# raznem/spp-rl

Hardware: AMD Instinct MI355X
Metric: env-steps/sec (rollout+update) SPP-SAC Hopper-v2 (higher is better)
Workload: dtype fp32

## Files before the change

include/spprl.h:

```cpp
#ifndef SPPRL_H
#define SPPRL_H
#include <stdint.h>

#ifdef __cplusplus
extern "C" {
#endif

typedef int sppStatus;
enum {
  SPP_OK = 0,
  SPP_E_INVALID_ARG = 1,
  SPP_E_SHAPE = 2,
  SPP_E_OOM = 3,
  SPP_E_HIP = 4,
  SPP_E_STATE = 5,
  SPP_E_RCCL = 6
};

const char* sppGetLastError(void);
int sppGetVersion(void);

typedef struct sppMT19937* sppMTHandle;
sppStatus sppMTCreate(sppMTHandle* out, uint32_t seed);
sppStatus sppMTRandint(sppMTHandle h, int64_t high, int64_t n, int64_t* out_host);
// ... 113 lines not shown
sppStatus sppDdpgAcmCriticGrads(sppAgentHandle h, const sppBatch* batch, float* losses_dev, void* stream);
sppStatus sppDdpgAcmCriticApply(sppAgentHandle h, void* stream);
sppStatus sppDdpgAcmActorGrads(sppAgentHandle h, float* losses_dev, void* stream);
sppStatus sppDdpgAcmActorApply(sppAgentHandle h, void* stream);

#define SPP_COMM_ID_BYTES 128
sppStatus sppCommGetUniqueId(void* uid_out);
sppStatus sppCommInitRank(void** comm_out, int nranks, const void* uid, int rank, int device);
sppStatus sppCommDestroy(void* comm);
enum { SPP_BUCKET_CRITIC = 0, SPP_BUCKET_ACTOR = 1, SPP_BUCKET_ACM = 2, SPP_BUCKET_ALL = 3 };
sppStatus sppAllReduceGrads(sppAgentHandle h, int bucket, int world, void* rccl_comm, void* stream);
sppStatus sppCommAllReduceSum(void* rccl_comm, void* buf_dev, int64_t count, int dtype, void* stream);
sppStatus sppCommAllGather(void* rccl_comm, const void* send_dev, void* recv_dev, int64_t bytes, void* stream);

sppStatus sppAcmRegressStep(sppAgentHandle h, const float* x, const float* y, int B, float* loss_dev,
                            void* stream);
sppStatus sppAcmRegressGrads(sppAgentHandle h, const float* x, const float* y, int B, float* loss_dev,
                             void* stream);
sppStatus sppAcmRegressApply(sppAgentHandle h, void* stream);
sppStatus sppAcmSgd(sppAgentHandle h, const float* x_dev, const float* y_dev, int nsteps, int bs, float* loss_sum,
                    void* stream);
sppStatus sppAcmSgdEpoch(sppAgentHandle h, const float* x_dev, const float* y_dev, int nrows, int bs,
                         float* loss_sum, void* stream);
sppStatus sppAcmSgdStatus(sppAgentHandle h, int* timed_out_host);
sppStatus sppAcmSgdStatusAsync(sppAgentHandle h, int* timed_out_pinned, void* stream);
int sppAcmSgdMaxBatch(sppAgentHandle h);
int sppAcmSgdWorkgroups(sppAgentHandle h, int bs);
sppStatus sppReplayGatherAcm(sppReplayHandle h, const int64_t* idx_dev, int B, float* x, float* y, void* stream);
sppStatus sppReplaySetAcmColumns(sppReplayHandle h, const int* cols_host, int n);

sppStatus sppAgentSetTiming(sppAgentHandle h, int enable);
sppStatus sppAgentStageSplit(sppAgentHandle h, int* bits_out);
sppStatus sppAgentCriticPairs(sppAgentHandle h, int* bits_out);
sppStatus sppAgentGetTiming(sppAgentHandle h, double* ms_out , int64_t* count_out );

sppStatus sppPolicyAct(sppAgentHandle h, const float* obs , int E, const float* eps ,
                       const float* noise , float act_noise, int mode, int denormalize_actor_out,
                       float* target_state_out , float* env_action_out , void* stream);

sppStatus sppSynthEnvStep(const float* A , const float* obs , const float* action ,
                          int E, int ob, int ac, float* next_obs, float* reward, void* stream);

sppStatus sppRandUniform(float* out_dev, int64_t n, const float* lo_dev, const float* hi_dev, int period,
                         uint64_t seed, uint64_t offset, void* stream);
sppStatus sppEpisodeAccum(const float* rew, const uint8_t* end, int E, float* ep_ret, double* sums, void* stream);
sppStatus sppSynthEnvReset(float* obs , const uint8_t* mask, int E, int ob, uint64_t seed,
                           uint64_t offset, void* stream);

sppStatus sppObsNormalize(const float* x, int64_t rows, int ob, const float* lo, const float* hi, const float* mean,
                          const float* std, int min_max, int inverse, float* out, void* stream);

sppStatus sppGaeScan(const float* rew, const float* v, const float* v_next, const uint8_t* done,
                     const uint8_t* end, int64_t T, int64_t E, double gamma, double lam, int mode, float* q_out,
                     float* adv, void* stream);
sppStatus sppPpoClipLoss(const float* lp_old, const float* lp_new, const float* adv, int B, float eps, float* grad,
                         float* out2, void* stream);
sppStatus sppAdvNormalize(const float* adv, int64_t n, float* out, void* stream);
sppStatus sppAdvSums(const float* adv, int64_t n, double* sums2, void* stream);
sppStatus sppAdvNormalizeGlobal(const float* adv, int64_t n_local, const double* sums2, int64_t n_global, float* out,
                                void* stream);

typedef struct sppOnPolicy* sppOnPolicyHandle;
typedef struct {
  int ob, aout;
  float actor_lr, critic_lr;
  float ppo_epsilon;
// ... 51 lines not shown
```

spp-rl_amd/csrc/api.hip:

```cpp
#include <dlfcn.h>
#include <stdarg.h>
#include <stdio.h>
#include <string.h>

#include <algorithm>
#include <memory>
#include <string>
#include <vector>

#include "../../include/spprl.h"
#include "internal.h"
#include "layout.h"
#include "replay.h"
#include "sac_kernels.h"
#include "host.h"

#include "optim.hip"
#include "replay.hip"
#include "stats.hip"
#include "sac.hip"
#include "ddpg.hip"
#include "kset.h"
#ifdef SPP_SINGLE_TU
#include "ks_dw.hip"
// ... 1026 lines not shown
    }
    D.j0[0] = 0;
    D.nj[0] = (int)jobs.size();
  }
  if (a->cfg.mlp_bf16) {
    std::vector<const float*> b16;
    if (!a->ddpg && set == 0)
      b16 = {a->H1[0], a->H1[1], a->H2[0], a->H2[1], a->D1[0], a->D1[1], a->D2[0], a->D2[1],
             a->AH1, a->AH2, a->AD1, a->AD2};
    auto is16 = [&](const float* p) { return p && std::find(b16.begin(), b16.end(), p) != b16.end(); };
    for (DwJob& j : jobs) {
      j.bf16 = 1;
      j.a_bf = is16(j.A) ? 1 : 0;
      j.x_bf = is16(j.X0) ? 1 : 0;
    }
  }
  const sppStatus s = finalize_dw(D, jobs, nph, Bp, B, a->num_cu);
  if (set == 0) {
    for (int i = 0; i < 2; ++i) {
      const int f = fused[a->ddpg ? 0 : i];
      a->w3p[i] = f >= 0 ? jobs[f].slab : nullptr;
    }
    a->w3p_stride = fused[0] >= 0 ? jobs[fused[0]].slab_stride : 0;
  }
  return s;
}

namespace spp {

void launch_dw_set(DwSet& D, int ph, hipStream_t st) {
  const int* ij = D.items.ptr + D.ioff[ph];
  const int* is = ij + D.nitems[ph];
  const DwJob* jobs = D.jobs.ptr + D.j0[ph];
  launch_dw_kernels(jobs, ij, is, D.nitems[ph], D.nlds[ph], D.nj[ph], D.max_elems[ph], D.bf16, st);
}

int g_sgd_spin = 0;

constexpr int kSgdSyncInts = kSgdShardStride * (1 + kSgdShards);
int* sgd_ctr(DevArray<int>& sync) { return sync.ptr + kSgdShardStride; }
sppStatus mlp_sgd_buffers(DevArray<float>& slab, DevArray<int>& sync, hipStream_t st) {
  if (!slab.ptr) {
    SPP_CHECK_HIP(slab.alloc((size_t)(2 * kMlMaxWG + kSgdPubReps) * kMlSlabMax));
    SPP_CHECK_HIP(sync.alloc(kSgdSyncInts));
    SPP_CHECK_HIP(hipMemsetAsync(sync.ptr, 0, kSgdSyncInts * sizeof(int), st));
  }
  SPP_CHECK_HIP(hipMemsetAsync(sgd_ctr(sync), 0, kSgdShards * kSgdShardStride * sizeof(int), st));
  return SPP_OK;
}

void launch_pack_matrix(int gx, int njobs, const PackJob* jobs, hipStream_t st) {
  hipLaunchKernelGGL(k_pack_matrix, dim3(gx, njobs), dim3(256), 0, st, jobs);
}
void launch_adam_kernel(const AdamJob* job, int64_t n, float neg_step, float bc2s, hipStream_t st) {
  hipLaunchKernelGGL(k_adam, dim3(std::max(1, std::min(cdiv(n, 1024), 1024)), 1), dim3(256), 0, st, job, neg_step,
                     bc2s, 0.f);
}

}

static void launch_dw(sppAgent* a, int set, int ph, hipStream_t st) { launch_dw_set(a->dws[set], ph, st); }

static sppStatus build_adam(sppAgent* a) {
  AdamJob jobs[4] = {};
  for (int i = 0; i < (a->ddpg ? 1 : 2); ++i) {
    NetBufs& n = a->net[SPP_NET_CRITIC1 + i];
    jobs[i] = AdamJob{n.p, n.g, n.m, n.v, a->net[SPP_NET_CRITIC1_TARG + i].p, n.n};
  }
  NetBufs& na = a->net[SPP_NET_ACTOR];
  jobs[2] = AdamJob{na.p, na.g, na.m, na.v, a->ddpg ? a->net[SPP_NET_ACTOR_TARG].p : nullptr, na.n};
  NetBufs& nm = a->net[SPP_NET_ACM];
  jobs[3] = AdamJob{nm.p, nm.g, nm.m, nm.v, nullptr, nm.n};
  if (!a->d_adam.ptr) SPP_CHECK_HIP(a->d_adam.alloc(4));
  SPP_CHECK_HIP(hipMemcpy(a->d_adam.ptr, jobs, sizeof(jobs), hipMemcpyHostToDevice));
  return SPP_OK;
}

static void launch_adam(sppAgent* a, int first, int count, int64_t n, int64_t step, float lr, float tau,
                        hipStream_t st) {
  const double bc1 = 1.0 - std::pow(0.9, (double)step), bc2s = std::sqrt(1.0 - std::pow(0.999, (double)step));
  hipLaunchKernelGGL(k_adam, dim3(std::max(1, std::min(cdiv(n, 256 * 4), 1024)), count), dim3(256), 0, st,
                     (const AdamJob*)(a->d_adam.ptr + first), (float)(-(lr / bc1)), (float)bc2s, tau);
}

constexpr int kStageWGPerCU = 3;
constexpr int kStageSplitAll = 7;
constexpr int kStageSplitDefault = kStageSplitAll;
constexpr int kCriticPairsDefault = 1;
static int stage_grid(sppAgent* a, int Bp) {
  return std::max(1, std::min(cdiv(Bp / 32, kWavesPerWG), kStageWGPerCU * a->num_cu));
}

static SacArgs make_args(sppAgent* a, int B) {
  SacArgs p{};
  p.B = B;
  p.Bp = (int)round_up(B, 32);
  p.inv_B = 1.f / (float)B;
  p.S = a->S; p.S2 = a->S2; p.ACT = a->ACT; p.AENV = a->AENV; p.R = a->R; p.DN = a->DN;
  p.EPS1 = a->EPS1; p.EPS2 = a->EPS2;
  p.min_max = a->cfg.min_max_denormalize;
  p.lo = a->lo; p.hi = a->hi; p.mean = a->mean; p.std = a->std;
  p.actor_lim = a->limits.ptr;
  p.acm_lim = a->limits.ptr + a->cfg.aout;
  p.gamma = a->cfg.gamma;
  p.custom_loss = a->cfg.custom_loss;
  p.norm_closs = a->cfg.norm_closs;
  p.alpha = a->alpha_f32;
  p.actor = a->actor;
  for (int i = 0; i < 2; ++i) {
    p.critic[i] = a->critic[i];
    p.targ[i] = a->targ[i];
    p.H1[i] = a->H1[i]; p.H2[i] = a->H2[i]; p.D1[i] = a->D1[i]; p.D2[i] = a->D2[i]; p.DQ[i] = a->DQ[i];
    p.W3P[i] = a->w3p[i];
  }
  p.w3p_stride = a->w3p_stride;
  p.acm = a->acm;
  p.bacm = a->bacm;
  p.actor_targ = a->actor_targ;
  p.AH1 = a->AH1; p.AH2 = a->AH2; p.AD1 = a->AD1; p.AD2 = a->AD2; p.ADH = a->ADH;
  p.part = a->part;
  p.THD = a->THD; p.SCA = a->SCA; p.SLP = a->SLP;
// ... 59 lines not shown
  SPP_REQUIRE(cfg->algo != SPP_ALGO_SAC || (cfg->acm_critic == 0 && cfg->aout == cfg->ac && cfg->custom_loss == 0.f),
              SPP_E_INVALID_ARG, "vanilla SAC: the actor emits the env action (aout == ac), no ACM critic / loss");
  SPP_REQUIRE(cfg->algo != SPP_ALGO_DDPG || (cfg->acm_critic == 0 && cfg->aout == cfg->ac && cfg->custom_loss == 0.f),
              SPP_E_INVALID_ARG, "vanilla DDPG: the actor emits the env action (aout == ac), no ACM critic / loss");
  SPP_REQUIRE(cfg->algo != SPP_ALGO_DDPG || cfg->mlp_bf16 == 0, SPP_E_INVALID_ARG, "vanilla DDPG: fp32 only");
  SPP_REQUIRE(cfg->max_batch > 0, SPP_E_INVALID_ARG, "max_batch must be > 0");
  KernelSet ks;
  SPP_REQUIRE(find_kset(cfg->algo, cfg->ob, cfg->aout, cfg->ac, cfg->acm_critic != 0, cfg->mlp_bf16 != 0, &ks),
              SPP_E_SHAPE, "no kernel instantiation for algo %d (ob=%d, aout=%d, ac=%d, bf16=%d)", cfg->algo, cfg->ob,
              cfg->aout, cfg->ac, cfg->mlp_bf16);
  SPP_CHECK_HIP(hipSetDevice(device));
  auto a = std::make_unique<sppAgent>();
  a->cfg = *cfg;
  a->device = device;
  a->ks = ks;
  hipDeviceProp_t prop;
  SPP_CHECK_HIP(hipGetDeviceProperties(&prop, device));
  a->num_cu = prop.multiProcessorCount;
  {
    const char* t = getenv("SPP_SAC_TEAM");
    a->team_ok = !(t && t[0] == '0');
    const char* m = getenv("SPP_MINQ_SPLIT");
    a->minq_split = ks.actor_fwd && ks.actor_minq && ks.actor_bwd && !(m && m[0] == '0');
    const char* g = getenv("SPP_STAGE_SPLIT");
    const int want = g ? atoi(g) : kStageSplitDefault;
    const bool tab_fits = 128 + 3 * round_up(std::max(cfg->aout, 1), 32) + round_up(std::max(cfg->ac, 1), 32) <= kStageTab;
    const bool have = ks.heads_stage && ks.trunk_bwd && ks.trunk_fwd_a && ks.squash_a && ks.critics_a &&
                      ks.trunk_fwd_c && ks.squash_c && ks.critic_rest;
    if (a->minq_split && have && tab_fits) a->stage_split = want & kStageSplitAll;
    const char* cp = getenv("SPP_CRITIC_PAIRS");
    const int wantp = cp ? atoi(cp) : kCriticPairsDefault;
    if ((a->stage_split & 4) && ks.critic_rest_pair) a->critic_pairs |= wantp & 1;
    if ((a->stage_split & 2) && ks.critics_a_pair) a->critic_pairs |= wantp & 2;
  }
  const int ob = cfg->ob, aout = cfg->aout, ac = cfg->ac;
  a->cin = ob + (cfg->acm_critic ? ac : aout);
  a->ddpg = cfg->algo == SPP_ALGO_DDPG_ACM || cfg->algo == SPP_ALGO_DDPG;
  a->plain = cfg->algo == SPP_ALGO_SAC || cfg->algo == SPP_ALGO_DDPG;
  const bool dd = a->ddpg;
  a->lay[SPP_NET_ACTOR] = dd ? ddpg_actor_layout(ob, aout) : sac_actor_layout(ob, aout);
  if (dd) a->lay[SPP_NET_ACTOR_TARG] = a->lay[SPP_NET_ACTOR];
  a->lay[SPP_NET_CRITIC1] = a->lay[SPP_NET_CRITIC1_TARG] = critic_layout(a->cin);
  if (!dd) a->lay[SPP_NET_CRITIC2] = a->lay[SPP_NET_CRITIC2_TARG] = critic_layout(a->cin);
  if (!dd) a->lay[SPP_NET_ACM] = acm_layout(2 * ob, ac);
  else if (!a->plain) a->lay[SPP_NET_ACM] = bacm_layout(2 * ob, ac);
  a->Bmax = cfg->max_batch;
  const int64_t Bp = round_up(cfg->max_batch, 32);
  SPP_REQUIRE((int64_t)Bp * 256 * 4 < ((int64_t)1 << 31), SPP_E_SHAPE, "max_batch %d too large (31-bit buffer offsets)",
              cfg->max_batch);
  a->Bpmax = (int)Bp;
  const int64_t ntiles = Bp / 32;
  const int64_t per = Bp;
  int64_t total = 0;
  auto take = [&](int64_t rows) { int64_t o = total; total += rows * per; return o; };
  const int64_t oS = take(ob), oS2 = take(ob), oACT = take(aout), oAENV = take(ac), oR = take(1), oDN = take(1),
                oE1 = take(aout), oE2 = take(aout);
  int64_t oH1[2] = {}, oH2[2] = {}, oD1[2] = {}, oD2[2] = {}, oDQ[2] = {};
  for (int i = 0; i < (dd ? 1 : 2); ++i) {
    oH1[i] = take(256); oH2[i] = take(256); oD1[i] = take(256); oD2[i] = take(256); oDQ[i] = take(1);
  }
  const int64_t oAH1 = take(256), oAH2 = take(256), oAD1 = take(256), oAD2 = take(256), oADH = take(2 * aout);
  const int64_t oZ1 = take(dd ? 128 : 64), oZ2 = take(dd ? 64 : 32), oT3 = take(ac);
  const int64_t oRX = take(2 * ob), oRZ1 = take(dd ? 128 : 64), oRZ2 = take(dd ? 64 : 32), oRP1 = take(dd ? 128 : 64),
                oRP2 = take(dd ? 64 : 32), oRP3 = take(ac);
  const int64_t oRS21 = dd ? take(64) : 0, oRPZ21 = dd ? take(64) : 0;
  const int64_t oGAD = take(aout), oMASK = take(16);
// ... 234 lines not shown
  }
  tmark(a, 1, st);
  SPP_CHECK_HIP(hipGetLastError());
  tmark(a, 2, st);
  launch_dw(a, 0, 1, st);
  tmark(a, 2, st);
  hipLaunchKernelGGL(k_actor_partials, dim3(1), dim3(kFinThreads), 0, st, (const float*)a->part, p.Bp / 32, B, a->cfg.aout,
                     a->cfg.custom_loss, (double)a->cfg.target_entropy, a->alpha_grad ? a->alpha_grad : a->aux,
                     losses);
  SPP_CHECK_HIP(hipGetLastError());
  return SPP_OK;
}

sppStatus sppSacAcmActorGrads(sppAgentHandle a, const float* eps_cur, float* losses, void* stream) {
  SPP_REQUIRE(a, SPP_E_INVALID_ARG, "null");
  const int B = a->cur_B;
  SPP_REQUIRE(B > 0, SPP_E_STATE, "no staged batch");
  const int Bp = (int)round_up(B, 32);
  if (eps_cur)
    hipLaunchKernelGGL(k_eps_copy_fm, dim3(cdiv((int64_t)a->cfg.aout * Bp, 256)), dim3(256), 0, S(stream), eps_cur,
                       a->EPS2, a->cfg.aout, B, Bp);
  return actor_grads(a, losses, S(stream));
}

sppStatus sppAgentStageSplit(sppAgentHandle a, int* bits_out) {
  SPP_REQUIRE(a && bits_out, SPP_E_INVALID_ARG, "null");
  *bits_out = a->stage_split;
  return SPP_OK;
}

sppStatus sppAgentCriticPairs(sppAgentHandle a, int* bits_out) {
  SPP_REQUIRE(a && bits_out, SPP_E_INVALID_ARG, "null");
  *bits_out = a->critic_pairs;
  return SPP_OK;
}

sppStatus sppAgentBindAlphaGrad(sppAgentHandle a, float* g) {
  SPP_REQUIRE(a, SPP_E_INVALID_ARG, "null");
  a->alpha_grad = g;
  return SPP_OK;
}

sppStatus sppSacAcmDrawEps(sppAgentHandle a, uint64_t seed, uint64_t counter, void* stream) {
  SPP_REQUIRE(a && a->cur_B > 0, SPP_E_STATE, "no staged batch");
  const int B = a->cur_B, Bp = (int)round_up(B, 32);
  SPP_REQUIRE((int64_t)a->cfg.aout * Bp < ((int64_t)1 << 31), SPP_E_SHAPE, "draw_eps: aout * Bp >= 2^31");
  const int64_t quads = (int64_t)a->cfg.aout * Bp / 4;
  hipLaunchKernelGGL(k_eps_fm, dim3(cdiv(quads, 256), 2), dim3(256), 0, S(stream), a->EPS1, a->cfg.aout, B, Bp, seed,
                     2 * counter, a->EPS2, 2 * counter + 1);
  SPP_CHECK_HIP(hipGetLastError());
  return SPP_OK;
}

sppStatus sppAgentReadEps(sppAgentHandle a, int which, float* out, void* stream) {
  SPP_REQUIRE(a && out && (which == 0 || which == 1), SPP_E_INVALID_ARG, "read_eps: bad args");
  SPP_REQUIRE(a->cur_B > 0, SPP_E_STATE, "no staged batch");
  const int B = a->cur_B, Bp = (int)round_up(B, 32);
  hipLaunchKernelGGL(k_eps_read_fm, dim3(cdiv((int64_t)a->cfg.aout * B, 256)), dim3(256), 0, S(stream),
                     (const float*)(which ? a->EPS2 : a->EPS1), out, a->cfg.aout, B, Bp);
  SPP_CHECK_HIP(hipGetLastError());
  return SPP_OK;
}

static std::vector<PackJob> images_of(sppAgent* a, int net) {
  std::vector<PackJob> out;
  const NetBufs& nb = a->net[net];
// ... 611 lines not shown
```

spp-rl_amd/csrc/dw.hip:

```cpp
#include "common.h"
#include "internal.h"

namespace spp {

constexpr int kDwThreads = 256;

template <int NI, int NJ, bool BF = false, bool ABF = false, bool XBF = false>
constexpr int dw_ring() {
  constexpr int cyc = NI * NJ * (BF ? 32 : 512);
  constexpr int want = 1 + (8192 + cyc - 1) / cyc;
  constexpr int cap = 168 / (4 * (NI * (ABF ? 1 : 2) + NJ * (XBF ? 1 : 2)));
  constexpr int r = want < cap ? want : cap;
  return r < 2 ? 2 : (r > 8 ? 8 : r);
}

__device__ __forceinline__ bf16x8 pack8(const float4& a, const float4& b) {
  bf16x8 r;
  r[0] = (__bf16)a.x; r[1] = (__bf16)a.y; r[2] = (__bf16)a.z; r[3] = (__bf16)a.w;
  r[4] = (__bf16)b.x; r[5] = (__bf16)b.y; r[6] = (__bf16)b.z; r[7] = (__bf16)b.w;
  return r;
}

__device__ __forceinline__ bf16x8 as_bf8(const float4& a) { return __builtin_bit_cast(bf16x8, a); }
__device__ __forceinline__ float sum_bf8(const float4& a) {
// ... 51 lines not shown
      if constexpr (BF) {
        static_for<0, NI>([&](auto I) {
          if constexpr (DB && ABF) {
            bs[I] += sum_bf8(ra[u][I][0]);
          } else if constexpr (DB) {
            const float4 a0 = ra[u][I][0], a1 = ra[u][I][1];
            bs[I] += ((a0.x + a0.y) + (a0.z + a0.w)) + ((a1.x + a1.y) + (a1.z + a1.w));
          }
          const bf16x8 av = ABF ? as_bf8(ra[u][I][0]) : pack8(ra[u][I][0], ra[u][I][1]);
          static_for<0, NJ>([&](auto J) {
            const bf16x8 xv = XBF ? as_bf8(rx[u][J][0]) : pack8(rx[u][J][0], rx[u][J][1]);
            acc[I][J] = mfma16(av, xv, acc[I][J]);
          });
        });
      } else {
        static_for<0, NI>([&](auto I) {
          static_for<0, 2>([&](auto P) {
            const float4 av = ra[u][I][P];
            if constexpr (DB) bs[I] += (av.x + av.y) + (av.z + av.w);
            static_for<0, NJ>([&](auto J) {
              const float4 xv = rx[u][J][P];
              acc[I][J] = mfma(av.x, xv.x, acc[I][J]);
              acc[I][J] = mfma(av.y, xv.y, acc[I][J]);
              acc[I][J] = mfma(av.z, xv.z, acc[I][J]);
              acc[I][J] = mfma(av.w, xv.w, acc[I][J]);
            });
          });
        });
      }
    });
  }
}

typedef __attribute__((address_space(1))) void glob_void;
typedef __attribute__((address_space(3))) void lds_void;
__device__ __forceinline__ void dw_big_lds(const DwJob& J, int b_begin, int nsteps, int nb0, int kb0, bool db,
                                           f32x16 (&acc)[4][4], float (&bs)[4]) {
  __shared__ __attribute__((aligned(16))) float lds[2][512 * 32];
  const int tid = threadIdx.x, w = tid >> 6, lane = tid & 63, h = lane >> 5, c = lane & 31;
  const int64_t ld = J.Bp;
  const int pe = (lane & 7) ^ ((lane >> 4) & 3);
  const int wu = __builtin_amdgcn_readfirstlane(w);
  const float* wsel = wu < 2 ? J.A : J.X0;
  const uint64_t wbits = (uint64_t)(size_t)wsel;
  const uint64_t wbu = (uint64_t)(uint32_t)__builtin_amdgcn_readfirstlane((int)(uint32_t)wbits) |
                       ((uint64_t)(uint32_t)__builtin_amdgcn_readfirstlane((int)(uint32_t)(wbits >> 32)) << 32);
  const int64_t ldu = (int64_t)__builtin_amdgcn_readfirstlane((int)ld);
  const int bbu = __builtin_amdgcn_readfirstlane(b_begin);
  const float* wb = opaque(reinterpret_cast<const float*>((size_t)wbu) + (int64_t)(128 * (wu & 1)) * ldu + bbu);
  const uint32_t off0 = (uint32_t)((lane >> 3) * ld + 4 * pe), off1 = off0 ^ 16u;
  auto issue = [&](int t, int buf) {
    const uint32_t dst = (uint32_t)(size_t)(lds_void*)&lds[buf][(128 * wu) * 32];
#pragma unroll
    for (int k = 0; k < 16; ++k) {
      const float* src = opaque(wb + ((int64_t)(8 * k) * ldu + 32 * t)) + ((k & 1) ? off1 : off0);
      uint32_t keep;
      asm volatile("s_mov_b32 %0, m0\n\ts_mov_b32 m0, %2\n\ts_nop 0\n\tglobal_load_lds_dwordx4 %1, off\n\ts_mov_b32 m0, %0"
                   : "=&s"(keep)
                   : "v"(src), "s"(dst + 1024u * k)
                   : "memory");
    }
  };
  const int sw = (c >> 1) & 7;
  auto rd = [&](const float* L, int s, float4 (&ra)[4][2], float4 (&rx)[4][2]) {
    const int q0 = (4 * s + 2 * h) ^ sw, q1 = (4 * s + 2 * h + 1) ^ sw;
#pragma unroll
// ... 4 lines not shown
      ra[i][1] = *reinterpret_cast<const float4*>(pa + 4 * q1);
      rx[i][0] = *reinterpret_cast<const float4*>(px + 4 * q0);
      rx[i][1] = *reinterpret_cast<const float4*>(px + 4 * q1);
    }
  };
  auto mm = [&](const float4 (&ra)[4][2], const float4 (&rx)[4][2]) {
#pragma unroll
    for (int i = 0; i < 4; ++i)
#pragma unroll
      for (int p = 0; p < 2; ++p) {
        const float4 av = ra[i][p];
        if (db) bs[i] += (av.x + av.y) + (av.z + av.w);
#pragma unroll
        for (int j = 0; j < 4; ++j) {
          const float4 xv = rx[j][p];
          acc[i][j] = mfma(av.x, xv.x, acc[i][j]);
          acc[i][j] = mfma(av.y, xv.y, acc[i][j]);
          acc[i][j] = mfma(av.z, xv.z, acc[i][j]);
          acc[i][j] = mfma(av.w, xv.w, acc[i][j]);
        }
      }
  };
  issue(0, 0);
  asm volatile("s_waitcnt vmcnt(0)" ::: "memory");
  __syncthreads();
  if (nsteps > 1) issue(1, 1);
  float4 ra0[4][2], rx0[4][2], ra1[4][2], rx1[4][2];
  rd(lds[0], 0, ra0, rx0);
#pragma unroll 1
  for (int t = 0; t < nsteps; ++t) {
    rd(lds[t & 1], 1, ra1, rx1);
    mm(ra0, rx0);
    if (t + 1 < nsteps) {
      asm volatile("s_waitcnt vmcnt(0) lgkmcnt(0)" ::: "memory");
      __syncthreads();
      if (t + 2 < nsteps) issue(t + 2, t & 1);
      rd(lds[(t + 1) & 1], 0, ra0, rx0);
    }
    mm(ra1, rx1);
  }
}

__device__ __forceinline__ void dw_big_lds16(const DwJob& J, int b_begin, int nsteps, int nb0, int kb0, bool db,
                                             f32x16 (&acc)[4][4], float (&bs)[4]) {
  __shared__ __attribute__((aligned(16))) float lds[2][512 * 32];
  const int tid = threadIdx.x, w = tid >> 6, lane = tid & 63, h = lane >> 5, c = lane & 31;
  const int64_t ld = J.Bp / 2;
  const int pe = (lane & 7) ^ ((lane >> 4) & 3);
  const int wu = __builtin_amdgcn_readfirstlane(w);
  const float* wsel = wu < 2 ? J.A : J.X0;
  const uint64_t wbits = (uint64_t)(size_t)wsel;
  const uint64_t wbu = (uint64_t)(uint32_t)__builtin_amdgcn_readfirstlane((int)(uint32_t)wbits) |
                       ((uint64_t)(uint32_t)__builtin_amdgcn_readfirstlane((int)(uint32_t)(wbits >> 32)) << 32);
  const int64_t ldu = (int64_t)__builtin_amdgcn_readfirstlane((int)ld);
  const int bbu = __builtin_amdgcn_readfirstlane(b_begin / 2);
  const float* wb = opaque(reinterpret_cast<const float*>((size_t)wbu) + (int64_t)(128 * (wu & 1)) * ldu + bbu);
  const uint32_t off0 = (uint32_t)((lane >> 3) * ld + 4 * pe), off1 = off0 ^ 16u;
  auto issue = [&](int t, int buf) {
    const uint32_t dst = (uint32_t)(size_t)(lds_void*)&lds[buf][(128 * wu) * 32];
#pragma unroll
    for (int k = 0; k < 16; ++k) {
      const float* src = opaque(wb + ((int64_t)(8 * k) * ldu + 32 * t)) + ((k & 1) ? off1 : off0);
      uint32_t keep;
      asm volatile("s_mov_b32 %0, m0\n\ts_mov_b32 m0, %2\n\ts_nop 0\n\tglobal_load_lds_dwordx4 %1, off\n\ts_mov_b32 m0, %0"
                   : "=&s"(keep)
                   : "v"(src), "s"(dst + 1024u * k)
                   : "memory");
    }
  };
  const int sw = (c >> 1) & 7;
  auto rd = [&](const float* L, int s, float4 (&ra)[4], float4 (&rx)[4]) {
    const int q = (2 * s + h) ^ sw;
// ... 7 lines not shown
#pragma unroll
    for (int i = 0; i < 4; ++i) {
      if (db) bs[i] += sum_bf8(ra[i]);
      const bf16x8 av = as_bf8(ra[i]);
#pragma unroll
      for (int j = 0; j < 4; ++j) acc[i][j] = mfma16(av, as_bf8(rx[j]), acc[i][j]);
    }
  };
  issue(0, 0);
  asm volatile("s_waitcnt vmcnt(0)" ::: "memory");
  __syncthreads();
  if (nsteps > 1) issue(1, 1);
  float4 ra0[4], rx0[4], ra1[4], rx1[4];
  rd(lds[0], 0, ra0, rx0);
#pragma unroll 1
  for (int t = 0; t < nsteps; ++t) {
    const float* L = lds[t & 1];
    rd(L, 1, ra1, rx1);
    mm(ra0, rx0);
    rd(L, 2, ra0, rx0);
    mm(ra1, rx1);
    rd(L, 3, ra1, rx1);
    mm(ra0, rx0);
    if (t + 1 < nsteps) {
      asm volatile("s_waitcnt vmcnt(0) lgkmcnt(0)" ::: "memory");
      __syncthreads();
      if (t + 2 < nsteps) issue(t + 2, t & 1);
      rd(lds[(t + 1) & 1], 0, ra0, rx0);
    }
    mm(ra1, rx1);
  }
}

__device__ __forceinline__ void dw_store(const DwJob& J, int split, int part, int nb0, int kb0, int ni, int nj,
                                         bool db, const f32x16 (&acc)[4][4], const float (&bs)[4]) {
  int tid = threadIdx.x;
  asm volatile("" : "+v"(nb0), "+v"(kb0), "+v"(ni), "+v"(nj), "+v"(split), "+v"(part), "+v"(tid));
  const int lane = tid & 63, h = lane >> 5, c = lane & 31;
  const int N = J.N, K = J.K0 + J.K1;
  const bool direct = J.nsplit * J.wsplit == 1;
  float* slab = direct ? nullptr : J.slab + (int64_t)(split * J.wsplit + part) * J.slab_stride;
  auto row_w = [&](int n) -> float* {
    if (!direct) return slab + (int64_t)n * K;
    return n < J.nrow2 ? J.dW + (int64_t)n * K : J.dW2 + (int64_t)(n - J.nrow2) * K;
  };
#pragma unroll
  for (int i = 0; i < 4; ++i) {
    if (i >= ni) break;
#pragma unroll
    for (int q = 0; q < 16; ++q) {
      const int n = 32 * (nb0 + i) + unit_of(q, h);
      if (n >= N) continue;
      float* rowp = row_w(n);
      asm volatile("" : "+v"(rowp));
#pragma unroll
      for (int j = 0; j < 4; ++j) {
        if (j >= nj) break;
        const int k = 32 * (kb0 + j) + c;
        if (k < K) rowp[k] = acc[i][j][q];
      }
    }
    if (db) {
      const float tot = bs[i] + __shfl_xor(bs[i], 32, 64);
      const int n = 32 * (nb0 + i) + c;
      if (h == 0 && n < N) {
        if (!direct) slab[(int64_t)N * K + n] = tot;
        else if (n < J.nrow2) J.db[n] = tot;
        else J.db2[n - J.nrow2] = tot;
      }
    }
  }
}

template <bool BFK>
__global__ __launch_bounds__(kDwThreads, 1) void k_dw(const DwJob* __restrict__ jobs, const int* __restrict__ item_job,
                                                      const int* __restrict__ item_split) {
  const int item = blockIdx.x;
  const DwJob J = jobs[item_job[item]];
  const int split = item_split[item];
  const int w = threadIdx.x >> 6, lane = threadIdx.x & 63, h = lane >> 5, c = lane & 31;
  const int64_t ld = J.Bp;
  const int N = J.N, K = J.K0 + J.K1;
  const bool wsp = J.wsplit > 1;
  int nb0 = 4 * (w >> 1), kb0 = 4 * (w & 1), part = 0;
  if (J.wsplit == 4) {
    nb0 = kb0 = 0;
    part = w;
  } else if (J.wsplit == 2) {
    if (N <= 128) {
// ... 133 lines not shown
  float s = 0.f;
  if (G == 1) {
    int sp = 0;
    for (; sp + 16 <= nslab; sp += 16) {
      float v[16];
#pragma unroll
      for (int u = 0; u < 16; ++u) v[u] = p[(int64_t)(sp + u) * J.slab_stride];
#pragma unroll
      for (int u = 0; u < 16; ++u) s += v[u];
    }
    for (; sp < nslab; ++sp) s += p[(int64_t)sp * J.slab_stride];
  } else {
    for (int sp = g; sp < nslab; sp += 16 * G) {
      float v[16];
#pragma unroll
      for (int u = 0; u < 16; ++u) v[u] = sp + u * G < nslab ? p[(int64_t)(sp + u * G) * J.slab_stride] : 0.f;
#pragma unroll
      for (int u = 0; u < 16; ++u) s += v[u];
    }
    for (int o = G / 2; o > 0; o >>= 1) s += __shfl_xor(s, o, 64);
    if (g != 0) return;
  }
  if (e < nw) {
    const int n = (int)(e / K), k = (int)(e % K);
    if (n < J.nrow2) J.dW[(int64_t)n * K + k] = s;
    else J.dW2[(int64_t)(n - J.nrow2) * K + k] = s;
  } else {
    const int n = (int)(e - nw);
    if (n < J.nrow2) J.db[n] = s;
    else J.db2[n - J.nrow2] = s;
  }
}

}
```

spp-rl_amd/csrc/host.h:

```cpp
#pragma once
#include <algorithm>
#include <vector>

#include "../../include/spprl.h"
#include "internal.h"
#include "layout.h"
#include "sac_kernels.h"
#include "sgd.hip"
#include "sgd_mlp.hip"

namespace spp {

static inline hipStream_t S(void* s) { return reinterpret_cast<hipStream_t>(s); }

struct NetBufs {
  float *p = nullptr, *g = nullptr, *m = nullptr, *v = nullptr;
  int64_t n = 0;
};

template <typename T>
struct DevArray {
  T* ptr = nullptr;
  size_t n = 0;
  hipError_t alloc(size_t count) {
    n = count;
    return hipMalloc(&ptr, sizeof(T) * std::max<size_t>(count, 1));
  }
  void release() {
    if (ptr) (void)hipFree(ptr);
    ptr = nullptr;
  }
};

struct DwSet {
  DevArray<float> slab;
  DevArray<DwJob> jobs;
  DevArray<int> items;
  int B = -1;
  int j0[2] = {0, 0}, nj[2] = {0, 0}, ioff[2] = {0, 0}, nitems[2] = {0, 0};
  int nlds[2] = {0, 0};
  int64_t max_elems[2] = {1, 1};
  bool bf16 = false;
  void release() { slab.release(); jobs.release(); items.release(); }
};

struct PackPlan {
  struct Image {
    int list;
    PackJob job;
    const float4** slot;
  };
  std::vector<Image> images;
  std::vector<TabSeg> tab;
  int toff = 0;
  int bf16 = 0;
  void M(int list, const float* W, const float* W2, int split, int ld, int trans, int coff, MapDesc out, MapDesc in,
         int NBO, int NBI, const float4** slot, int ib = 0) {
    images.push_back({list, PackJob{W, W2, split, ld, trans, coff, out, in, NBO, NBI, ib, nullptr, bf16}, slot});
  }
  int T(const float* v, int n, const float* v2 = nullptr, int n2 = 0) {
    const int off = toff, tot = (int)round_up(n + n2, 32);
    tab.push_back(TabSeg{v, n, v2 ? n : tot, off, 0});
    if (v2) tab.push_back(TabSeg{v2, n2, tot - n, off + n, 0});
    toff += tot;
    return off;
  }
  sppStatus commit(int nlists, DevArray<float4>& pk, DevArray<PackJob>& d_pj, std::vector<PackJob>& jobs, int* off) {
    size_t nf4 = 0;
    for (auto& m : images) nf4 += (size_t)m.job.NBO * m.job.NBI * 4 * 64;
    pk.release();
    SPP_CHECK_HIP(pk.alloc(nf4));
    size_t of = 0;
    for (auto& m : images) {
      m.job.dst = pk.ptr + of;
      *m.slot = m.job.dst;
// ... 44 lines not shown
```

spp-rl_amd/csrc/internal.h:

```cpp
#pragma once
#include "common.h"
#include "mlp.h"

namespace spp {

struct DwJob {
  const float* A;
  const float* X0;
  const float* X1;
  float* dW;
  float* db;
  float* dW2;
  float* db2;
  float* slab;
  int64_t slab_stride;
  int N, K0, K1, Bp;
  int split_len, nsplit, nrow2;
  int wsplit;
  int bf16;
  int a_bf, x_bf;
  int fused;
};

void launch_dw_kernels(const DwJob* jobs, const int* item_job, const int* item_split, int nitems, int nlds,
                       int njobs, int64_t max_elems, bool bf16, hipStream_t st);
inline __host__ __device__ int dw_red_group(int nslab, int64_t elems) { return nslab >= 64 && elems <= 4096 ? 16 : 1; }

struct PackJob {
  const float* W;
  const float* W2;
  int split, ld, trans, coff;
  MapDesc out, in;
  int NBO, NBI, ibmajor;
  float4* dst;
  int bf16;
};

struct AdamJob {
  float* p;
  const float* g;
  float* m;
  float* v;
  float* targ;
  int64_t n;
};

}
```

spp-rl_amd/csrc/ks_dw.hip:

```cpp
#include "dw.hip"

namespace spp {
void launch_dw_kernels(const DwJob* jobs, const int* item_job, const int* item_split, int nitems, int nlds,
                       int njobs, int64_t max_elems, bool bf16, hipStream_t st) {
  if (nlds > 0)
    hipLaunchKernelGGL(bf16 ? k_dw_big16 : k_dw_big, dim3(nlds), dim3(kDwThreads), 0, st, jobs, item_job, item_split);
  if (nitems > nlds)
    hipLaunchKernelGGL(bf16 ? k_dw<true> : k_dw<false>, dim3(nitems - nlds), dim3(kDwThreads), 0, st, jobs,
                       item_job + nlds, item_split + nlds);
  hipLaunchKernelGGL(k_dw_reduce, dim3(cdiv(max_elems, 256), njobs), dim3(256), 0, st, jobs);
}
}
```

spp-rl_amd/spprl/_lib.py:

```python
import ctypes
import os

import torch

HERE = os.path.dirname(os.path.abspath(__file__))
LIB_PATH = os.environ.get("SPPRL_LIB") or os.path.join(HERE, "libspprl.so")

(SPP_NET_ACTOR, SPP_NET_CRITIC1, SPP_NET_CRITIC2, SPP_NET_CRITIC1_TARG, SPP_NET_CRITIC2_TARG, SPP_NET_ACM,
 SPP_NET_ACTOR_TARG) = range(7)
SPP_ALGO_SAC_ACM, SPP_ALGO_DDPG_ACM, SPP_ALGO_SAC, SPP_ALGO_DDPG = 1, 2, 3, 4
SPP_BUCKET_CRITIC, SPP_BUCKET_ACTOR, SPP_BUCKET_ACM, SPP_BUCKET_ALL = range(4)
SPP_COMM_ID_BYTES = 128
SPP_DP1_REUSE_BRACKET = 0x100
NUM_LOSSES = 8

c_int, c_int64, c_uint32, c_uint64, c_float, c_void_p = (ctypes.c_int, ctypes.c_int64, ctypes.c_uint32,
                                                         ctypes.c_uint64, ctypes.c_float, ctypes.c_void_p)


class SppError(RuntimeError):
    pass


class AgentConfig(ctypes.Structure):
# ... 52 lines not shown
    "sppAgentCreate": (c_int, [P(c_void_p), P(AgentConfig), c_int]),
    "sppAgentDestroy": (c_int, [c_void_p]),
    "sppAgentNetSize": (c_int, [c_void_p, c_int, P(c_int64)]),
    "sppAgentBindNet": (c_int, [c_void_p, c_int, c_void_p, c_void_p, c_void_p, c_void_p]),
    "sppAgentSetLimits": (c_int, [c_void_p, c_void_p, c_void_p]),
    "sppAgentBindNormalizer": (c_int, [c_void_p, c_void_p, c_void_p, c_void_p, c_void_p]),
    "sppAgentBindAlpha": (c_int, [c_void_p, c_void_p, c_void_p]),
    "sppAgentSetSteps": (c_int, [c_void_p, c_int64, c_int64, c_int64, c_int64]),
    "sppAgentGetSteps": (c_int, [c_void_p, c_void_p]),
    "sppSacAcmUpdate": (c_int, [c_void_p, P(Batch), c_void_p, c_void_p, c_void_p, c_void_p]),
    "sppSacAcmCriticGrads": (c_int, [c_void_p, P(Batch), c_void_p, c_void_p, c_void_p]),
    "sppSacAcmCriticApply": (c_int, [c_void_p, c_void_p]),
    "sppSacAcmActorGrads": (c_int, [c_void_p, c_void_p, c_void_p, c_void_p]),
    "sppSacAcmActorApply": (c_int, [c_void_p, c_void_p, c_void_p]),
    "sppAgentStageFromReplay": (c_int, [c_void_p, c_void_p, c_void_p, c_int, c_void_p]),
    "sppAgentStagePost": (c_int, [c_void_p, c_int, c_int, c_void_p]),
    "sppSacAcmUpdateStaged": (c_int, [c_void_p, c_uint64, c_uint64, c_void_p, c_void_p]),
    "sppAcmRegressStep": (c_int, [c_void_p, c_void_p, c_void_p, c_int, c_void_p, c_void_p]),
    "sppPolicyAct": (c_int, [c_void_p, c_void_p, c_int, c_void_p, c_void_p, c_float, c_int, c_int, c_void_p,
                             c_void_p, c_void_p]),
    "sppAgentBindAlphaGrad": (c_int, [c_void_p, c_void_p]),
    "sppSacAcmDrawEps": (c_int, [c_void_p, c_uint64, c_uint64, c_void_p]),
    "sppAgentReadEps": (c_int, [c_void_p, c_int, c_void_p, c_void_p]),
    "sppAgentImageCount": (c_int, [c_void_p, c_int, c_void_p]),
    "sppAgentUnpackImage": (c_int, [c_void_p, c_int, c_int, c_void_p, c_void_p]),
    "sppAcmRegressGrads": (c_int, [c_void_p, c_void_p, c_void_p, c_int, c_void_p, c_void_p]),
    "sppAcmRegressApply": (c_int, [c_void_p, c_void_p]),
    "sppReplayGatherAcm": (c_int, [c_void_p, c_void_p, c_int, c_void_p, c_void_p, c_void_p]),
    "sppReplaySetAcmColumns": (c_int, [c_void_p, c_void_p, c_int]),
    "sppAgentSetTiming": (c_int, [c_void_p, c_int]),
    "sppAgentGetTiming": (c_int, [c_void_p, c_void_p, c_void_p]),
    "sppAgentStageSplit": (c_int, [c_void_p, P(c_int)]),
    "sppAgentCriticPairs": (c_int, [c_void_p, P(c_int)]),
    "sppSynthEnvStep": (c_int, [c_void_p, c_void_p, c_void_p, c_int, c_int, c_int, c_void_p, c_void_p, c_void_p]),
    "sppDdpgAcmUpdate": (c_int, [c_void_p, P(Batch), c_void_p, c_void_p]),
    "sppDdpgAcmCriticGrads": (c_int, [c_void_p, P(Batch), c_void_p, c_void_p]),
    "sppDdpgAcmCriticApply": (c_int, [c_void_p, c_void_p]),
    "sppDdpgAcmActorGrads": (c_int, [c_void_p, c_void_p, c_void_p]),
    "sppDdpgAcmActorApply": (c_int, [c_void_p, c_void_p]),
    "sppOnpCreate": (c_int, [P(c_void_p), P(OnPolicyConfig), c_int]),
    "sppOnpDestroy": (c_int, [c_void_p]),
    "sppOnpNetSize": (c_int, [c_void_p, c_int, P(c_int64)]),
    "sppOnpBindNet": (c_int, [c_void_p, c_int, c_void_p, c_void_p, c_void_p, c_void_p]),
    "sppOnpSetLimits": (c_int, [c_void_p, c_void_p]),
    "sppOnpValue": (c_int, [c_void_p, c_void_p, c_int, c_void_p, c_void_p]),
    "sppOnpCriticGrads": (c_int, [c_void_p, c_void_p, c_void_p, c_int, c_void_p, c_void_p]),
    "sppOnpCriticApply": (c_int, [c_void_p, c_void_p]),
    "sppOnpActorGrads": (c_int, [c_void_p, c_void_p, c_void_p, c_void_p, c_void_p, c_void_p, c_int, c_void_p,
                                 c_void_p]),
    "sppOnpActorApply": (c_int, [c_void_p, c_void_p]),
    "sppOnpTdAdvantage": (c_int, [c_void_p, c_void_p, c_void_p, c_void_p, c_void_p, c_int, c_float, c_void_p,
                                  c_void_p, c_void_p, c_void_p]),
    "sppOnpPgActorGrads": (c_int, [c_void_p] * 7 + [c_int, c_void_p, c_void_p]),
    "sppOnpAct": (c_int, [c_void_p, c_void_p, c_int, c_void_p, c_void_p, c_void_p, c_void_p]),
    "sppOnpRolloutAct": (c_int, [c_void_p, c_void_p, c_int, c_void_p, c_void_p, c_uint64, c_uint64, c_int, c_void_p,
                                 c_void_p, c_void_p, c_void_p, c_void_p]),
    "sppOnpObsStats": (c_int, [c_void_p, c_int64, c_void_p, c_int64, c_void_p, c_int64, c_int, ctypes.c_double,
                               c_void_p, c_void_p, c_void_p, c_void_p, c_int, c_void_p]),
    "sppGaeScan": (c_int, [c_void_p, c_void_p, c_void_p, c_void_p, c_void_p, c_int64, c_int64, ctypes.c_double,
                           ctypes.c_double,
                            c_int, c_void_p, c_void_p, c_void_p]),
    "sppPpoClipLoss": (c_int, [c_void_p, c_void_p, c_void_p, c_int, c_float, c_void_p, c_void_p, c_void_p]),
    "sppAdvNormalize": (c_int, [c_void_p, c_int64, c_void_p, c_void_p]),
    "sppRandUniform": (c_int, [c_void_p, c_int64, c_void_p, c_void_p, c_int, c_uint64, c_uint64, c_void_p]),
    "sppEpisodeAccum": (c_int, [c_void_p, c_void_p, c_int, c_void_p, c_void_p, c_void_p]),
    "sppSynthEnvReset": (c_int, [c_void_p, c_void_p, c_int, c_int, c_uint64, c_uint64, c_void_p]),
# ... 73 lines not shown
```

Measured before the change: 469,400.

## Add 8-wave fp32 weight-gradient kernel with split async LDS loads

Adds k_dw_big8, a 512-thread variant of the large weight-gradient (dW) kernel. Each wave owns a 4x2 tile of MFMA accumulators instead of 4x4, and the global-to-LDS copies are split across two wave groups that issue at different points in the loop. It is selected by default for fp32 and can be switched back to the 4-wave kernel with SPP_DW_BIG_WAVES. The aim is more waves and more latency hiding per dW item. The cost is fewer workgroups per CU, since launch bounds allow one, plus extra LDS traffic per MFMA.

```diff
diff --git a/include/spprl.h b/include/spprl.h
--- a/include/spprl.h
+++ b/include/spprl.h
@@ -169,6 +169,7 @@
 sppStatus sppAgentSetTiming(sppAgentHandle h, int enable);
 sppStatus sppAgentStageSplit(sppAgentHandle h, int* bits_out);
 sppStatus sppAgentCriticPairs(sppAgentHandle h, int* bits_out);
+sppStatus sppAgentDwBigWaves(sppAgentHandle h, int* waves_out);
 sppStatus sppAgentGetTiming(sppAgentHandle h, double* ms_out , int64_t* count_out );
 
 sppStatus sppPolicyAct(sppAgentHandle h, const float* obs , int E, const float* eps ,
diff --git a/spp-rl_amd/csrc/api.hip b/spp-rl_amd/csrc/api.hip
--- a/spp-rl_amd/csrc/api.hip
+++ b/spp-rl_amd/csrc/api.hip
@@ -1082,7 +1082,7 @@
   const int* ij = D.items.ptr + D.ioff[ph];
   const int* is = ij + D.nitems[ph];
   const DwJob* jobs = D.jobs.ptr + D.j0[ph];
-  launch_dw_kernels(jobs, ij, is, D.nitems[ph], D.nlds[ph], D.nj[ph], D.max_elems[ph], D.bf16, st);
+  launch_dw_kernels(jobs, ij, is, D.nitems[ph], D.nlds[ph], D.nj[ph], D.max_elems[ph], D.bf16, D.big_waves, st);
 }
 
 int g_sgd_spin = 0;
@@ -1137,6 +1137,7 @@
 constexpr int kStageSplitAll = 7;
 constexpr int kStageSplitDefault = kStageSplitAll;
 constexpr int kCriticPairsDefault = 1;
+constexpr int kDwBigWavesDefault = 8;
 static int stage_grid(sppAgent* a, int Bp) {
   return std::max(1, std::min(cdiv(Bp / 32, kWavesPerWG), kStageWGPerCU * a->num_cu));
 }
@@ -1262,6 +1263,9 @@
     const int wantp = cp ? atoi(cp) : kCriticPairsDefault;
     if ((a->stage_split & 4) && ks.critic_rest_pair) a->critic_pairs |= wantp & 1;
     if ((a->stage_split & 2) && ks.critics_a_pair) a->critic_pairs |= wantp & 2;
+    const char* bw = getenv("SPP_DW_BIG_WAVES");
+    const int wantw = bw ? atoi(bw) : kDwBigWavesDefault;
+    for (DwSet& D : a->dws) D.big_waves = wantw == 8 && !cfg->mlp_bf16 ? 8 : 4;
   }
   const int ob = cfg->ob, aout = cfg->aout, ac = cfg->ac;
   a->cin = ob + (cfg->acm_critic ? ac : aout);
@@ -1562,6 +1566,12 @@
 sppStatus sppAgentCriticPairs(sppAgentHandle a, int* bits_out) {
   SPP_REQUIRE(a && bits_out, SPP_E_INVALID_ARG, "null");
   *bits_out = a->critic_pairs;
+  return SPP_OK;
+}
+
+sppStatus sppAgentDwBigWaves(sppAgentHandle a, int* waves_out) {
+  SPP_REQUIRE(a && waves_out, SPP_E_INVALID_ARG, "null");
+  *waves_out = a->dws[0].big_waves;
   return SPP_OK;
 }
 
diff --git a/spp-rl_amd/csrc/dw.hip b/spp-rl_amd/csrc/dw.hip
--- a/spp-rl_amd/csrc/dw.hip
+++ b/spp-rl_amd/csrc/dw.hip
@@ -107,6 +107,9 @@
   }
 }
 
+#ifndef SPP_DW_TIMING
+#define SPP_DW_TIMING 0
+#endif
 typedef __attribute__((address_space(1))) void glob_void;
 typedef __attribute__((address_space(3))) void lds_void;
 __device__ __forceinline__ void dw_big_lds(const DwJob& J, int b_begin, int nsteps, int nb0, int kb0, bool db,
@@ -177,12 +180,99 @@
     rd(lds[t & 1], 1, ra1, rx1);
     mm(ra0, rx0);
     if (t + 1 < nsteps) {
+#if !(SPP_DW_TIMING & 2)
       asm volatile("s_waitcnt vmcnt(0) lgkmcnt(0)" ::: "memory");
       __syncthreads();
+#endif
+#if !(SPP_DW_TIMING & 1)
       if (t + 2 < nsteps) issue(t + 2, t & 1);
+#endif
       rd(lds[(t + 1) & 1], 0, ra0, rx0);
     }
     mm(ra1, rx1);
+  }
+}
+
+__device__ __forceinline__ void dw_big8_lds(const DwJob& J, int b_begin, int nsteps, int nb0, int kb0, bool db,
+                                            f32x16 (&acc)[4][2], float (&bs)[4]) {
+  __shared__ __attribute__((aligned(16))) float lds[2][512 * 32];
+  const int tid = threadIdx.x, w = tid >> 6, lane = tid & 63, h = lane >> 5, c = lane & 31;
+  const int64_t ld = J.Bp;
+  const int pe = (lane & 7) ^ ((lane >> 4) & 3);
+  const int wu = __builtin_amdgcn_readfirstlane(w);
+  const float* wsel = wu < 4 ? J.A : J.X0;
+  const uint64_t wbits = (uint64_t)(size_t)wsel;
+  const uint64_t wbu = (uint64_t)(uint32_t)__builtin_amdgcn_readfirstlane((int)(uint32_t)wbits) |
+                       ((uint64_t)(uint32_t)__builtin_amdgcn_readfirstlane((int)(uint32_t)(wbits >> 32)) << 32);
+  const int64_t ldu = (int64_t)__builtin_amdgcn_readfirstlane((int)ld);
+  const int bbu = __builtin_amdgcn_readfirstlane(b_begin);
+  const float* wb = opaque(reinterpret_cast<const float*>((size_t)wbu) + (int64_t)(64 * (wu & 3)) * ldu + bbu);
+  const uint32_t off0 = (uint32_t)((lane >> 3) * ld + 4 * pe), off1 = off0 ^ 16u;
+  const bool late = wu >= 4;
+  auto issue = [&](int t, int buf) {
+    const uint32_t dst = (uint32_t)(size_t)(lds_void*)&lds[buf][(64 * wu) * 32];
+#pragma unroll
+    for (int k = 0; k < 8; ++k) {
+      const float* src = opaque(wb + ((int64_t)(8 * k) * ldu + 32 * t)) + ((k & 1) ? off1 : off0);
+      uint32_t keep;
+      asm volatile("s_mov_b32 %0, m0\n\ts_mov_b32 m0, %2\n\ts_nop 0\n\tglobal_load_lds_dwordx4 %1, off\n\ts_mov_b32 m0, %0"
+                   : "=&s"(keep)
+                   : "v"(src), "s"(dst + 1024u * k)
+                   : "memory");
+    }
+  };
+  const int sw = (c >> 1) & 7;
+  auto rd = [&](const float* L, int v, float4 (&ra)[4], float4 (&rx)[2]) {
+    const int q = (4 * (v >> 1) + 2 * h + (v & 1)) ^ sw;
+#pragma unroll
+    for (int i = 0; i < 4; ++i) ra[i] = *reinterpret_cast<const float4*>(L + (32 * (nb0 + i) + c) * 32 + 4 * q);
+#pragma unroll
+    for (int j = 0; j < 2; ++j) rx[j] = *reinterpret_cast<const float4*>(L + (256 + 32 * (kb0 + j) + c) * 32 + 4 * q);
+  };
+  auto mm = [&](const float4 (&ra)[4], const float4 (&rx)[2]) {
+#pragma unroll
+    for (int i = 0; i < 4; ++i) {
+      const float4 av = ra[i];
+      if (db) bs[i] += (av.x + av.y) + (av.z + av.w);
+#pragma unroll
+      for (int j = 0; j < 2; ++j) {
+        const float4 xv = rx[j];
+        acc[i][j] = mfma(av.x, xv.x, acc[i][j]);
+        acc[i][j] = mfma(av.y, xv.y, acc[i][j]);
+        acc[i][j] = mfma(av.z, xv.z, acc[i][j]);
+        acc[i][j] = mfma(av.w, xv.w, acc[i][j]);
+      }
+    }
+  };
+  issue(0, 0);
+  asm volatile("s_waitcnt vmcnt(0)" ::: "memory");
+  __syncthreads();
+  if (nsteps > 1) issue(1, 1);
+  float4 ra0[4], rx0[2], ra1[4], rx1[2];
+  rd(lds[0], 0, ra0, rx0);
+#pragma unroll 1
+  for (int t = 0; t < nsteps; ++t) {
+    const float* L = lds[t & 1];
+    rd(L, 1, ra1, rx1);
+    mm(ra0, rx0);
+    rd(L, 2, ra0, rx0);
+    mm(ra1, rx1);
+    rd(L, 3, ra1, rx1);
+    mm(ra0, rx0);
+    if (t + 1 < nsteps) {
+#if !(SPP_DW_TIMING & 2)
+      asm volatile("s_waitcnt vmcnt(0) lgkmcnt(0)" ::: "memory");
+      __syncthreads();
+#endif
+#if !(SPP_DW_TIMING & 1)
+      if (!late && t + 2 < nsteps) issue(t + 2, t & 1);
+#endif
+      rd(lds[(t + 1) & 1], 0, ra0, rx0);
+    }
+    mm(ra1, rx1);
+#if !(SPP_DW_TIMING & 1)
+    if (late && t + 2 < nsteps) issue(t + 2, t & 1);
+#endif
   }
 }
 
@@ -256,8 +346,9 @@
   }
 }
 
+template <int NJ = 4>
 __device__ __forceinline__ void dw_store(const DwJob& J, int split, int part, int nb0, int kb0, int ni, int nj,
-                                         bool db, const f32x16 (&acc)[4][4], const float (&bs)[4]) {
+                                         bool db, const f32x16 (&acc)[4][NJ], const float (&bs)[4]) {
   int tid = threadIdx.x;
   asm volatile("" : "+v"(nb0), "+v"(kb0), "+v"(ni), "+v"(nj), "+v"(split), "+v"(part), "+v"(tid));
   const int lane = tid & 63, h = lane >> 5, c = lane & 31;
@@ -278,7 +369,7 @@
       float* rowp = row_w(n);
       asm volatile("" : "+v"(rowp));
 #pragma unroll
-      for (int j = 0; j < 4; ++j) {
+      for (int j = 0; j < NJ; ++j) {
         if (j >= nj) break;
         const int k = 32 * (kb0 + j) + c;
         if (k < K) rowp[k] = acc[i][j][q];
@@ -478,4 +569,28 @@
   }
 }
 
-}
+constexpr int kDwBig8Threads = 512;
+template <int = 0>
+__global__ __launch_bounds__(kDwBig8Threads, 1) void k_dw_big8(const DwJob* __restrict__ jobs,
+                                                               const int* __restrict__ item_job,
+                                                               const int* __restrict__ item_split) {
+  const int item = blockIdx.x;
+  const DwJob J = jobs[item_job[item]];
+  const int split = item_split[item];
+  const int w = threadIdx.x >> 6;
+  const int nb0 = 4 * ((w >> 1) & 1), kb0 = 4 * (w & 1) + 2 * (w >> 2);
+  const int b_begin = split * J.split_len;
+  const int b_end = min(b_begin + J.split_len, J.Bp);
+  const int nsteps = (b_end - b_begin) / 32;
+  const bool db = J.db != nullptr && kb0 == 0;
+  f32x16 acc[4][2];
+#pragma unroll
+  for (int i = 0; i < 4; ++i)
+#pragma unroll
+    for (int j = 0; j < 2; ++j) acc[i][j] = zero16();
+  float bs[4] = {0.f, 0.f, 0.f, 0.f};
+  if (nsteps > 0) dw_big8_lds(J, b_begin, nsteps, nb0, kb0, db, acc, bs);
+  dw_store<2>(J, split, 0, nb0, kb0, 4, 2, db, acc, bs);
+}
+
+}
diff --git a/spp-rl_amd/csrc/host.h b/spp-rl_amd/csrc/host.h
--- a/spp-rl_amd/csrc/host.h
+++ b/spp-rl_amd/csrc/host.h
@@ -41,6 +41,7 @@
   int nlds[2] = {0, 0};
   int64_t max_elems[2] = {1, 1};
   bool bf16 = false;
+  int big_waves = 4;
   void release() { slab.release(); jobs.release(); items.release(); }
 };
 
diff --git a/spp-rl_amd/csrc/internal.h b/spp-rl_amd/csrc/internal.h
--- a/spp-rl_amd/csrc/internal.h
+++ b/spp-rl_amd/csrc/internal.h
@@ -23,7 +23,7 @@
 };
 
 void launch_dw_kernels(const DwJob* jobs, const int* item_job, const int* item_split, int nitems, int nlds,
-                       int njobs, int64_t max_elems, bool bf16, hipStream_t st);
+                       int njobs, int64_t max_elems, bool bf16, int big_waves, hipStream_t st);
 inline __host__ __device__ int dw_red_group(int nslab, int64_t elems) { return nslab >= 64 && elems <= 4096 ? 16 : 1; }
 
 struct PackJob {
diff --git a/spp-rl_amd/csrc/ks_dw.hip b/spp-rl_amd/csrc/ks_dw.hip
--- a/spp-rl_amd/csrc/ks_dw.hip
+++ b/spp-rl_amd/csrc/ks_dw.hip
@@ -2,12 +2,18 @@
 
 namespace spp {
 void launch_dw_kernels(const DwJob* jobs, const int* item_job, const int* item_split, int nitems, int nlds,
-                       int njobs, int64_t max_elems, bool bf16, hipStream_t st) {
-  if (nlds > 0)
-    hipLaunchKernelGGL(bf16 ? k_dw_big16 : k_dw_big, dim3(nlds), dim3(kDwThreads), 0, st, jobs, item_job, item_split);
+                       int njobs, int64_t max_elems, bool bf16, int big_waves, hipStream_t st) {
+  const auto thin = bf16 ? k_dw<true> : k_dw<false>;
+  if (nlds > 0) {
+    if (bf16)
+      hipLaunchKernelGGL(k_dw_big16, dim3(nlds), dim3(kDwThreads), 0, st, jobs, item_job, item_split);
+    else if (big_waves == 8)
+      hipLaunchKernelGGL(k_dw_big8<>, dim3(nlds), dim3(kDwBig8Threads), 0, st, jobs, item_job, item_split);
+    else
+      hipLaunchKernelGGL(k_dw_big, dim3(nlds), dim3(kDwThreads), 0, st, jobs, item_job, item_split);
+  }
   if (nitems > nlds)
-    hipLaunchKernelGGL(bf16 ? k_dw<true> : k_dw<false>, dim3(nitems - nlds), dim3(kDwThreads), 0, st, jobs,
-                       item_job + nlds, item_split + nlds);
+    hipLaunchKernelGGL(thin, dim3(nitems - nlds), dim3(kDwThreads), 0, st, jobs, item_job + nlds, item_split + nlds);
   hipLaunchKernelGGL(k_dw_reduce, dim3(cdiv(max_elems, 256), njobs), dim3(256), 0, st, jobs);
 }
 }
diff --git a/spp-rl_amd/spprl/_lib.py b/spp-rl_amd/spprl/_lib.py
--- a/spp-rl_amd/spprl/_lib.py
+++ b/spp-rl_amd/spprl/_lib.py
@@ -108,6 +108,7 @@
     "sppAgentGetTiming": (c_int, [c_void_p, c_void_p, c_void_p]),
     "sppAgentStageSplit": (c_int, [c_void_p, P(c_int)]),
     "sppAgentCriticPairs": (c_int, [c_void_p, P(c_int)]),
+    "sppAgentDwBigWaves": (c_int, [c_void_p, P(c_int)]),
     "sppSynthEnvStep": (c_int, [c_void_p, c_void_p, c_void_p, c_int, c_int, c_int, c_void_p, c_void_p, c_void_p]),
     "sppDdpgAcmUpdate": (c_int, [c_void_p, P(Batch), c_void_p, c_void_p]),
     "sppDdpgAcmCriticGrads": (c_int, [c_void_p, P(Batch), c_void_p, c_void_p]),
```

Result: faster. 475,800 (median of 6 runs) (+1.4%).
